# numz/ComfyUI-SeedVR2_VideoUpscaler

Hardware: AMD Instinct MI355X
Metric: upscaled frames/sec (720p->4K, SeedVR2-3B) (higher is better)
Workload: dtype bf16; 1 GPU; cfg3: SeedVR2-3B 32-frame 720p->4K clip (padded to 33 = 4n+1 for encode + DiT, 32 decoded), VAE tiled 1024/128; vae_tiled=True, parallelism=dp1, weights=random-init SeedVR2-3B + video_vae_v3 architecture (seeded)

## Files before the change

### comfyui-seedvr2_videoupscaler_amd/csrc/svr_conv_sub.hip

```cpp
#include "svr_common.h"
#include "../../include/seedvr2_hip.h"
#include <type_traits>

namespace svr {

constexpr int CS_TY = 16, CS_TX = 32, CS_HX = CS_TX + 1, CS_HY = CS_TY + 1;
constexpr int CS_NT = 256;
constexpr int CS_ROWS = CS_HX * CS_HY;
constexpr int CS_PIECES = (CS_ROWS * 4 + CS_NT - 1) / CS_NT;
constexpr int CS_ABUF = CS_PIECES * CS_NT * 16;
constexpr int CS_NBUF = 4;
constexpr int CS_EP_PITCH = 528;
constexpr int CS_EP_BYTES = 4 * 32 * CS_EP_PITCH;
constexpr int CS_LDS = CS_NBUF * CS_ABUF;
static_assert(CS_PIECES == 9 && CS_EP_BYTES <= CS_LDS, "piece schedule / epilogue parking");

template <int OFF> SVR_DEVICE void cs_rd2(bf16x8 (&r)[2], unsigned a0) {
    const unsigned a1 = a0 ^ 32u;
    asm volatile("ds_read_b128 %0, %2 offset:%4\n\tds_read_b128 %1, %3 offset:%4"
                 : "=&v"(r[0]), "=&v"(r[1]) : "v"(a0), "v"(a1), "n"(OFF) : "memory");
}
template <int N> SVR_DEVICE void cs_wait_rows(bf16x8 (&a)[2]) {
    asm volatile("s_waitcnt lgkmcnt(%2)" : "+v"(a[0]), "+v"(a[1]) : "n"(N));
    __builtin_amdgcn_sched_barrier(0);
}
template <int N> SVR_DEVICE void cs_wait_rows(bf16x8 (&a)[2], bf16x8 (&b)[2]) {
    asm volatile("s_waitcnt lgkmcnt(%4)" : "+v"(a[0]), "+v"(a[1]), "+v"(b[0]), "+v"(b[1]) : "n"(N));
    __builtin_amdgcn_sched_barrier(0);
}
template <int N> SVR_DEVICE void cs_wait_rows(bf16x8 (&a)[2], bf16x8 (&b)[2], bf16x8 (&c)[2], bf16x8 (&d)[2], bf16x8 (&e)[2]) {
    asm volatile("s_waitcnt lgkmcnt(%10)"
                 : "+v"(a[0]), "+v"(a[1]), "+v"(b[0]), "+v"(b[1]), "+v"(c[0]), "+v"(c[1]), "+v"(d[0]), "+v"(d[1]), "+v"(e[0]), "+v"(e[1])
                 : "n"(N));
    __builtin_amdgcn_sched_barrier(0);
}
template <int N> SVR_DEVICE void cs_wait_w(bf16x8 (&w)[2][2]) {
    asm volatile("s_waitcnt vmcnt(%4)" : "+v"(w[0][0]), "+v"(w[0][1]), "+v"(w[1][0]), "+v"(w[1][1]) : "n"(N));
    __builtin_amdgcn_sched_barrier(0);
}

__global__ __launch_bounds__(CS_NT, 1) void conv_sub_kernel(const svr_gemm_args a, const int band_rows) {
    constexpr int MTW = 8, NTW = 2, NT = CS_NT;
    extern __shared__ __attribute__((aligned(16))) char smem[];
    typedef __attribute__((ext_vector_type(16))) float f32x16_t;
    const svr_conv_geom& g = a.conv;
    const int tid = threadIdx.x;
    const int lane = tid & 63;
    const int wave = __builtin_amdgcn_readfirstlane(tid >> 6);
    const int wm = wave >> 1, wn = wave & 1;

    const int tiles_x = (g.W + CS_TX - 1) / CS_TX;
    const int tiles_y = (g.H + CS_TY - 1) / CS_TY;
    const int tiles_n = a.N / 128;
    int tl;
    {
        const int nwg = gridDim.x, bid = blockIdx.x;
        const int xcd = bid & 7, j = bid >> 3, q = nwg >> 3, r = nwg & 7;
        tl = (xcd < r ? xcd * (q + 1) : r * (q + 1) + (xcd - r) * q) + j;
    }
    const bool quad = a.phase.enabled && a.phase.quad != 0;
    int qp = 0;
    if (quad) { qp = tl & 3; tl >>= 2; }
    const int ph_py = quad ? (qp >> 1) : a.phase.py, ph_px = quad ? (qp & 1) : a.phase.px;
    const int pad_h = quad ? 1 - ph_py : g.ph, pad_w = quad ? 1 - ph_px : g.pw;
    const void* const w_frag = quad ? a.phase.W_frag4[qp] : a.W_frag;
    const float* const bias_p = quad ? a.phase.bias4[qp] : a.bias;
    const float* const bias_border_p = quad ? a.phase.bias_border4[qp] : a.phase.bias_border;
    const int tn = tl % tiles_n;
    int rr = tl / tiles_n;
    const int tx = rr % tiles_x; rr /= tiles_x;
    int ty, to;
    if (band_rows > 0 && band_rows < tiles_y) {
        const int per_band = band_rows * g.To;
        const int b = rr / per_band;
        const int rows_b = min(band_rows, tiles_y - b * band_rows);
        const int r2 = rr - b * per_band;
        to = r2 / rows_b;
        ty = b * band_rows + (r2 - to * rows_b);
    } else {
        ty = rr % tiles_y;
        to = rr / tiles_y;
    }
    const int y0 = ty * CS_TY, x0 = tx * CS_TX, n0 = tn * 128;

    const int cpk = g.Cin / 32;
    const int nA = g.kt * cpk;
    const int P = nA * 4;
    const int64_t frame_bytes = (int64_t)g.H * g.W * g.Cin * 2;
    const int srow = tid >> 2, spos = tid & 3;
    uint32_t poff[CS_PIECES];
    uint32_t akeys = 0;
#pragma unroll
    for (int q = 0; q < CS_PIECES; ++q) {
        const int row = q * (NT / 4) + srow;
        const int hy = row / CS_HX, hx = row - hy * CS_HX;
        const int y = y0 - pad_h + hy, x = x0 - pad_w + hx;
        const bool ok = (row < CS_ROWS) & ((unsigned)y < (unsigned)g.H) & ((unsigned)x < (unsigned)g.W);
        poff[q] = ok ? (uint32_t)(y * g.W + x) : 0xffffffffu;
        akeys |= (uint32_t)(spos ^ ((hx >> 2) & 3)) << (2 * q);
    }
    char* const wave_dst = smem + wave * 1024;
    auto frame_ptr = [&](int s) -> const char* {
        if (s >= nA) return nullptr;
        const int dt = s / cpk;
        const int c0 = (s - dt * cpk) * 32;
        int f = to + dt - g.pt;
        const char* basep = (const char*)a.A;
        if (f < 0) {
            if (g.halo != nullptr) { basep = (const char*)g.halo; f += g.halo_frames; }
            else f = 0;
        }
        return basep + (int64_t)f * frame_bytes + c0 * 2;
    };
    auto stage = [&](auto qc, const char* fptr, int buf) {
        constexpr int Q = decltype(qc)::value;
        const int ck = (akeys >> (2 * Q)) & 3;
        const char* src = (poff[Q] == 0xffffffffu || fptr == nullptr) ? (const char*)g.zeros
                                                                      : fptr + ((int64_t)poff[Q] * g.Cin + ck * 8) * 2;
        glds16(src, wave_dst + buf * CS_ABUF + Q * (NT * 16));
    };
    auto stage_all = [&](const char* fptr, int buf) {
        stage(std::integral_constant<int, 0>{}, fptr, buf); stage(std::integral_constant<int, 1>{}, fptr, buf);
        stage(std::integral_constant<int, 2>{}, fptr, buf); stage(std::integral_constant<int, 3>{}, fptr, buf);
        stage(std::integral_constant<int, 4>{}, fptr, buf); stage(std::integral_constant<int, 5>{}, fptr, buf);
        stage(std::integral_constant<int, 6>{}, fptr, buf); stage(std::integral_constant<int, 7>{}, fptr, buf);
        stage(std::integral_constant<int, 8>{}, fptr, buf);
    };

    const int l31 = lane & 31, hi = lane >> 5;
    const unsigned lds0 = (unsigned)(uintptr_t)(__attribute__((address_space(3))) char*)smem;
    unsigned fa[2];
#pragma unroll
    for (int dx = 0; dx < 2; ++dx)
        fa[dx] = lds0 + (unsigned)((wm * MTW * CS_HX + l31) * 64 + ((hi ^ (((dx + l31) >> 2) & 3)) << 4));

    f32x16_t acc[MTW][NTW];
#pragma unroll
    for (int y = 0; y < MTW; ++y)
#pragma unroll
        for (int z = 0; z < NTW; ++z)
#pragma unroll
            for (int e = 0; e < 16; ++e) acc[y][z][e] = 0.f;
    bf16x8 a0[2], a1[2], a2[2], a3[2], a4[2], a5[2], a6[2], a7[2], a8[2];
    bf16x8 w0[NTW][2], w1[NTW][2], w2[NTW][2], w3[NTW][2];

    const int64_t nstride = (int64_t)P * 2048;
    const char* wp0 = (const char*)w_frag + (int64_t)(n0 / 32 + wn * 2) * nstride;
    const char* wp1 = wp0 + nstride;
    const int voff = lane * 16;
    auto wload = [&](bf16x8 (&w)[NTW][2], int k) {
        auto uniform_ptr = [](const char* p) {
            const uint64_t u = (uint64_t)p;
            const uint32_t lo = __builtin_amdgcn_readfirstlane((uint32_t)u), hi_ = __builtin_amdgcn_readfirstlane((uint32_t)(u >> 32));
            return (const char*)(((uint64_t)hi_ << 32) | lo);
        };
        const char* p0 = uniform_ptr(wp0 + (int64_t)min(k, P - 1) * 2048);
        const char* p1 = uniform_ptr(wp1 + (int64_t)min(k, P - 1) * 2048);
        asm volatile("global_load_dwordx4 %0, %1, %2" : "=v"(w[0][0]) : "v"(voff), "s"(p0) : "memory");
        asm volatile("global_load_dwordx4 %0, %1, %2 offset:1024" : "=v"(w[0][1]) : "v"(voff), "s"(p0) : "memory");
        asm volatile("global_load_dwordx4 %0, %1, %2" : "=v"(w[1][0]) : "v"(voff), "s"(p1) : "memory");
        asm volatile("global_load_dwordx4 %0, %1, %2 offset:1024" : "=v"(w[1][1]) : "v"(voff), "s"(p1) : "memory");
    };

#define CS_RD(ROW, R, DXV, BUFOFF) cs_rd2<((R) * CS_HX + (DXV)) * 64>(ROW, fa[DXV] + (BUFOFF))
#define CS_MM(W, KS, ROW, MT, NTI) \
    acc[MT][NTI] = __builtin_amdgcn_mfma_f32_32x32x16_bf16(W[NTI][KS], ROW[KS], acc[MT][NTI], 0, 0, 0)
#define CS_MM8(W, RA, MA, RB, MB) \
    CS_MM(W, 0, RA, MA, 0); CS_MM(W, 0, RA, MA, 1); CS_MM(W, 0, RB, MB, 0); CS_MM(W, 0, RB, MB, 1); \
    CS_MM(W, 1, RA, MA, 0); CS_MM(W, 1, RA, MA, 1); CS_MM(W, 1, RB, MB, 0); CS_MM(W, 1, RB, MB, 1)

    auto interval = [&](auto jc, int s, const char* fstage, bf16x8 (&wc)[NTW][2], bf16x8 (&wn_)[NTW][2]) {
        constexpr int J = decltype(jc)::value;
        constexpr int DX = J >> 1, DY = J & 1;
        constexpr int NPC[4] = {0, 0, 5, 4};
        constexpr int NV = 4 + NPC[(J + 3) & 3] + NPC[(J + 2) & 3];
        const int k = s * 4 + J;
        const unsigned cur = (unsigned)((s & 3) * CS_ABUF), nxt = (unsigned)(((s + 1) & 3) * CS_ABUF);
        const int sbuf = (s + 3) & 3;
        constexpr int NDX = DX ^ 1;
        const unsigned nb = DX == 0 ? cur : nxt;
        if constexpr (DY == 0) {
            CS_RD(a8, 8, DX, cur);
            cs_wait_rows<8>(a0, a1, a2, a3, a4);
            cs_wait_w<NV>(wc);
            CS_MM8(wc, a0, 0, a1, 1);
            __builtin_amdgcn_sched_barrier(0);
            CS_RD(a0, 0, NDX, nb);
            wload(wn_, k + 2);
            __builtin_amdgcn_sched_barrier(0);
            CS_MM8(wc, a2, 2, a3, 3);
            __builtin_amdgcn_sched_barrier(0);
            if constexpr (J == 2) {
                stage(std::integral_constant<int, 0>{}, fstage, sbuf); stage(std::integral_constant<int, 1>{}, fstage, sbuf);
                stage(std::integral_constant<int, 2>{}, fstage, sbuf);
            }
            cs_wait_rows<8>(a4, a5);
            CS_MM8(wc, a4, 4, a5, 5);
            __builtin_amdgcn_sched_barrier(0);
            if constexpr (J == 2) { stage(std::integral_constant<int, 3>{}, fstage, sbuf); stage(std::integral_constant<int, 4>{}, fstage, sbuf); }
            cs_wait_rows<4>(a6, a7);
            CS_MM8(wc, a6, 6, a7, 7);
            __builtin_amdgcn_sched_barrier(0);
        } else {
            cs_wait_w<NV>(wc);
            CS_MM8(wc, a1, 0, a2, 1);
            __builtin_amdgcn_sched_barrier(0);
            CS_RD(a1, 1, NDX, nb); CS_RD(a2, 2, NDX, nb);
            wload(wn_, k + 2);
            __builtin_amdgcn_sched_barrier(0);
            CS_MM8(wc, a3, 2, a4, 3);
            __builtin_amdgcn_sched_barrier(0);
            CS_RD(a3, 3, NDX, nb); CS_RD(a4, 4, NDX, nb);
            if constexpr (J == 3) { stage(std::integral_constant<int, 5>{}, fstage, sbuf); stage(std::integral_constant<int, 6>{}, fstage, sbuf); }
            __builtin_amdgcn_sched_barrier(0);
            CS_MM8(wc, a5, 4, a6, 5);
            __builtin_amdgcn_sched_barrier(0);
            CS_RD(a5, 5, NDX, nb); CS_RD(a6, 6, NDX, nb);
            if constexpr (J == 3) { stage(std::integral_constant<int, 7>{}, fstage, sbuf); stage(std::integral_constant<int, 8>{}, fstage, sbuf); }
            cs_wait_rows<14>(a8);
            CS_MM8(wc, a7, 6, a8, 7);
            __builtin_amdgcn_sched_barrier(0);
            CS_RD(a7, 7, NDX, nb);
            if constexpr (J == 1) {
                __builtin_amdgcn_s_barrier();
                __builtin_amdgcn_sched_barrier(0);
            }
        }
    };

    stage_all(frame_ptr(0), 0);
    stage_all(frame_ptr(1), 1);
    stage_all(frame_ptr(2), 2);
    wload(w0, 0);
    wload(w1, 1);
    __builtin_amdgcn_sched_barrier(0);
#pragma unroll
    for (int y = 0; y < MTW; ++y)
#pragma unroll
        for (int z = 0; z < NTW; ++z) asm volatile("" : "+a"(acc[y][z]));
    asm volatile("s_waitcnt vmcnt(0)" ::: "memory");
    __builtin_amdgcn_s_barrier();
    __builtin_amdgcn_sched_barrier(0);
    CS_RD(a0, 0, 0, 0u); CS_RD(a1, 1, 0, 0u); CS_RD(a2, 2, 0, 0u); CS_RD(a3, 3, 0, 0u);
    CS_RD(a4, 4, 0, 0u); CS_RD(a5, 5, 0, 0u); CS_RD(a6, 6, 0, 0u); CS_RD(a7, 7, 0, 0u);

    for (int s = 0; s < nA; ++s) {
        const char* fs = frame_ptr(s + 3);
        interval(std::integral_constant<int, 0>{}, s, fs, w0, w2);
        interval(std::integral_constant<int, 1>{}, s, fs, w1, w3);
        interval(std::integral_constant<int, 2>{}, s, fs, w2, w0);
        interval(std::integral_constant<int, 3>{}, s, fs, w3, w1);
    }
    asm volatile("s_waitcnt vmcnt(0) lgkmcnt(0)" ::: "memory");
    __builtin_amdgcn_sched_barrier(0);
    __syncthreads();
#undef CS_RD
#undef CS_MM
#undef CS_MM8

    const int hi4 = hi * 4;
    const int n = n0 + (tid & 15) * 8;
    f32x4 bias_lo = {0.f, 0.f, 0.f, 0.f}, bias_hi = {0.f, 0.f, 0.f, 0.f};
    if (bias_p) {
        bias_lo = *(const f32x4*)(bias_p + n);
        bias_hi = *(const f32x4*)(bias_p + n + 4);
    }
    const int py = a.phase.enabled ? ph_py : 0, px = a.phase.enabled ? ph_px : 0;
    const int up = a.phase.enabled ? 2 : 1, ts = a.phase.enabled ? a.phase.t_stride : 1;
    const int yb = py ? g.H - 1 : 0, xb = px ? g.W - 1 : 0;
    const float* btab = a.phase.enabled ? bias_border_p : nullptr;
    double gs0 = 0.0, gq0 = 0.0, gs1 = 0.0, gq1 = 0.0;
    auto ep_body = [&](auto o32c) {
    constexpr int OKIND = decltype(o32c)::value;
    constexpr bool O32 = OKIND == SVR_STORE_FP32;
#pragma unroll
    for (int pass = 0; pass < MTW / 2; ++pass) {
        __builtin_amdgcn_sched_barrier(0);
#pragma unroll
        for (int j = 0; j < 2; ++j) {
            char* row = smem + ((wm * 2 + j) * 32 + l31) * CS_EP_PITCH;
#pragma unroll
            for (int nt = 0; nt < NTW; ++nt) {
                const f32x16_t v = acc[2 * pass + j][nt];
#pragma unroll
                for (int gq = 0; gq < 4; ++gq) {
                    const f32x4 o = {v[4 * gq], v[4 * gq + 1], v[4 * gq + 2], v[4 * gq + 3]};
                    *(f32x4*)(row + (wn * 64 + nt * 32 + 8 * gq + hi4) * 4) = o;
                }
            }
        }
        lds_barrier();
#pragma unroll
        for (int half = 0; half < 2; ++half) {
            f32x4 lo[4], hi_[4];
            int64_t off[4];
            bool ok[4];
            int border[4];
#pragma unroll
            for (int it = 0; it < 4; ++it) {
                const int vox = ((half * 4 + it) * NT + tid) >> 4;
                const int r = vox >> 5;
                const int y = y0 + (r >> 1) * MTW + 2 * pass + (r & 1), x = x0 + (vox & 31);
                ok[it] = y < g.H && x < g.W;
                const int yc = min(y, g.H - 1), xc = min(x, g.W - 1);
                border[it] = (yc == yb ? 1 : 0) | (xc == xb ? 2 : 0);
                off[it] = (((int64_t)to * ts * (up * g.H) + up * yc + py) * (up * g.W) + up * xc + px) * a.N + n;
                lo[it] = *(const f32x4*)(smem + vox * CS_EP_PITCH + (tid & 15) * 32);
                hi_[it] = *(const f32x4*)(smem + vox * CS_EP_PITCH + (tid & 15) * 32 + 16);
            }
#pragma unroll
            for (int it = 0; it < 4; ++it) {
                f32x4 bl = bias_lo, bh = bias_hi;
                if (btab != nullptr && border[it] != 0) {
                    const float* bb = btab + (int64_t)(border[it] - 1) * a.N + n;
                    bl = *(const f32x4*)bb;
                    bh = *(const f32x4*)(bb + 4);
                }
                const float f[8] = {lo[it][0] + bl[0], lo[it][1] + bl[1], lo[it][2] + bl[2], lo[it][3] + bl[3],
                                    hi_[it][0] + bh[0], hi_[it][1] + bh[1], hi_[it][2] + bh[2], hi_[it][3] + bh[3]};
                float r[8];
                if constexpr (O32) {
                    if (ok[it]) {
                        float* cp = (float*)a.C + off[it];
                        *(float4*)cp = make_float4(f[0], f[1], f[2], f[3]);
                        *(float4*)(cp + 4) = make_float4(f[4], f[5], f[6], f[7]);
                    }
#pragma unroll
                    for (int e = 0; e < 8; ++e) r[e] = f[e];
                } else {
                    const uint4 pk = OKIND == SVR_STORE_H16 ? pack8h(f) : pack8(f);
                    if (ok[it]) *(uint4*)((bf16_t*)a.C + off[it]) = pk;
                    if constexpr (OKIND == SVR_STORE_H16) unpack8h(pk, r); else unpack8(pk, r);
                }
                if (a.gn_partial != nullptr && ok[it]) {
                    gn_accumulate4(gs0, gq0, r[0], r[1], r[2], r[3]);
                    gn_accumulate4(gs1, gq1, r[4], r[5], r[6], r[7]);
                }
            }
        }
        if (pass + 1 < MTW / 2) lds_barrier();
    }
    };
    if (a.out_f32 == SVR_STORE_FP32) ep_body(std::integral_constant<int, SVR_STORE_FP32>{});
    else if (a.out_f32 == SVR_STORE_H16) ep_body(std::integral_constant<int, SVR_STORE_H16>{});
    else ep_body(std::integral_constant<int, SVR_STORE_BF16>{});
    if (a.gn_partial) {
        __syncthreads();
        double4* red = (double4*)smem;
        double2* qsum = (double2*)(smem + NT * 32);
        red[tid] = make_double4(gs0, gq0, gs1, gq1);
        __syncthreads();
        if (tid < 32) {
            const int c = tid >> 1, h = tid & 1;
            double s_ = 0.0, q_ = 0.0;
            for (int j = 0; j < NT / 16; ++j) {
                const double4 v = red[(j << 4) | c];
                s_ += h ? v.z : v.x;
                q_ += h ? v.w : v.y;
            }
            qsum[tid] = make_double2(s_, q_);
        }
        __syncthreads();
        const int qpg = (a.N / a.gn_groups) >> 2;
        if (tid < 32 / qpg) {
            double s_ = 0.0, q_ = 0.0;
            for (int i = 0; i < qpg; ++i) { s_ += qsum[tid * qpg + i].x; q_ += qsum[tid * qpg + i].y; }
            const int nblk = tiles_y * tiles_x;
            const int per_frame = a.phase.enabled ? 4 * nblk : nblk;
            const int slot = (a.phase.enabled ? (py * 2 + px) * nblk : 0) + ty * tiles_x + tx;
            ((double2*)a.gn_partial)[((int64_t)to * ts * per_frame + slot) * a.gn_groups + (n0 >> 2) / qpg + tid] = make_double2(s_, q_);
        }
    }
}

int g_conv_sub = 1;

static bool conv_sub_gn_ok(const svr_gemm_args& a) {
    const int cpg = a.gn_groups > 0 ? a.N / a.gn_groups : 0;
    return cpg >= 4 && !(cpg & 3) && a.N % a.gn_groups == 0 && 128 % cpg == 0;
}

static bool conv_sub_eligible(const svr_gemm_args& a) {
    const svr_conv_geom& g = a.conv;
    const bool quad = a.phase.enabled && a.phase.quad != 0;
    bool ptrs = true;
    if (quad) {
        for (int p = 0; p < 4; ++p)
            ptrs = ptrs && a.phase.W_frag4[p] != nullptr && (!a.phase.bias4[p] || ((uintptr_t)a.phase.bias4[p] % 16) == 0) &&
                   (!a.phase.bias_border4[p] || ((uintptr_t)a.phase.bias_border4[p] % 16) == 0);
    } else {
        ptrs = a.W_frag != nullptr && (unsigned)g.ph <= 1u && (unsigned)g.pw <= 1u && (!a.bias || ((uintptr_t)a.bias % 16) == 0) &&
               (!a.phase.bias_border || ((uintptr_t)a.phase.bias_border % 16) == 0);
    }
    return g_conv_sub && g.enabled && ptrs && g.kh == 2 && g.kw == 2 && g.sh == 1 && g.sw == 1 && g.st == 1 &&
           g.Ho == g.H && g.Wo == g.W && g.Cin % 32 == 0 && g.kt >= 1 && g.kt <= 3 &&
           g.To == g.T + g.pt - g.kt + 1 && !a.ps.enabled && a.epilogue == SVR_EPI_BIAS && !a.resid && !a.gate &&
           (!a.gn_partial || conv_sub_gn_ok(a)) && (a.N % 128) == 0 && (a.phase.enabled || (a.ldc == a.N)) &&
           (int64_t)g.H * g.W * g.Cin * 2 < (int64_t)1 << 32 && ((uintptr_t)a.C % 16) == 0;
}

static int conv_sub_gn_blocks(const svr_gemm_args& a) {
    if (!conv_sub_eligible(a) || !conv_sub_gn_ok(a)) return 0;
    const int nblk = ((a.conv.H + CS_TY - 1) / CS_TY) * ((a.conv.W + CS_TX - 1) / CS_TX);
    return a.phase.enabled ? 4 * nblk : nblk;
}

static int launch_conv_sub(const svr_gemm_args& a, hipStream_t s) {
    const svr_conv_geom& g = a.conv;
    const int tiles = g.To * ((g.H + CS_TY - 1) / CS_TY) * ((g.W + CS_TX - 1) / CS_TX) * (a.N / 128) *
                      (a.phase.enabled && a.phase.quad ? 4 : 1);
    static uint64_t lds_attr_done = 0;
    {
        const int e = set_max_dynamic_lds((const void*)conv_sub_kernel, 160 * 1024, lds_attr_done);
        if (e != 0) return e;
    }
    hipLaunchKernelGGL(conv_sub_kernel, dim3(tiles), dim3(CS_NT), CS_LDS, s, a, g_conv_band);
    return (int)hipGetLastError();
}

__global__ __launch_bounds__(256) void conv_pack_frag_taps_kernel(const bf16_t* __restrict__ W, uint4* __restrict__ out, int N, int K,
                                                                  int kt, int kh, int kw, int Cin) {
    const int cpk = Cin / 32, taps = kh * kw, P = kt * cpk * taps;
    const int64_t idx = (int64_t)blockIdx.x * 256 + threadIdx.x;
    if (idx >= (int64_t)(N / 32) * P * 128) return;
    const int lane = (int)(idx & 63), ks = (int)((idx >> 6) & 1);
    const int kk = (int)((idx >> 7) % P), n32 = (int)((idx >> 7) / P);
    const int s = kk / taps, J = kk - s * taps;
    const int dt = s / cpk, cs = s - dt * cpk, dy = J % kh, dx = J / kh;
    const int nn = n32 * 32 + (lane & 31), c = cs * 32 + ks * 16 + (lane >> 5) * 8;
    out[idx] = *(const uint4*)(W + (int64_t)nn * K + ((dt * kh + dy) * kw + dx) * Cin + c);
}

}
```

Before: 3.827 frames/s.

## Switch conv_sub inner product from 32x32x16 to 16x16x32 MFMA tiles

```diff
diff --git a/comfyui-seedvr2_videoupscaler_amd/csrc/svr_conv_sub.hip b/comfyui-seedvr2_videoupscaler_amd/csrc/svr_conv_sub.hip
--- a/comfyui-seedvr2_videoupscaler_amd/csrc/svr_conv_sub.hip
+++ b/comfyui-seedvr2_videoupscaler_amd/csrc/svr_conv_sub.hip
@@ -16,9 +16,15 @@
 static_assert(CS_PIECES == 9 && CS_EP_BYTES <= CS_LDS, "piece schedule / epilogue parking");
 
 template <int OFF> SVR_DEVICE void cs_rd2(bf16x8 (&r)[2], unsigned a0) {
-    const unsigned a1 = a0 ^ 32u;
-    asm volatile("ds_read_b128 %0, %2 offset:%4\n\tds_read_b128 %1, %3 offset:%4"
-                 : "=&v"(r[0]), "=&v"(r[1]) : "v"(a0), "v"(a1), "n"(OFF) : "memory");
+    static_assert(OFF >= 0 && OFF + 1024 + 16 <= 65536, "ds_read offset field");
+    asm volatile("ds_read_b128 %0, %2 offset:%3\n\tds_read_b128 %1, %2 offset:%4"
+                 : "=&v"(r[0]), "=&v"(r[1]) : "v"(a0), "n"(OFF), "n"(OFF + 1024) : "memory");
+}
+SVR_DEVICE void cs_mm4(f32x4 (&c)[2][2], const bf16x8 (&w)[2], const bf16x8 (&r)[2]) {
+    c[0][0] = __builtin_amdgcn_mfma_f32_16x16x32_bf16(w[0], r[0], c[0][0], 0, 0, 0);
+    c[0][1] = __builtin_amdgcn_mfma_f32_16x16x32_bf16(w[1], r[0], c[0][1], 0, 0, 0);
+    c[1][0] = __builtin_amdgcn_mfma_f32_16x16x32_bf16(w[0], r[1], c[1][0], 0, 0, 0);
+    c[1][1] = __builtin_amdgcn_mfma_f32_16x16x32_bf16(w[1], r[1], c[1][1], 0, 0, 0);
 }
 template <int N> SVR_DEVICE void cs_wait_rows(bf16x8 (&a)[2]) {
     asm volatile("s_waitcnt lgkmcnt(%2)" : "+v"(a[0]), "+v"(a[1]) : "n"(N));
@@ -42,7 +48,6 @@
 __global__ __launch_bounds__(CS_NT, 1) void conv_sub_kernel(const svr_gemm_args a, const int band_rows) {
     constexpr int MTW = 8, NTW = 2, NT = CS_NT;
     extern __shared__ __attribute__((aligned(16))) char smem[];
-    typedef __attribute__((ext_vector_type(16))) float f32x16_t;
     const svr_conv_geom& g = a.conv;
     const int tid = threadIdx.x;
     const int lane = tid & 63;
@@ -127,27 +132,27 @@
         stage(std::integral_constant<int, 8>{}, fptr, buf);
     };
 
-    const int l31 = lane & 31, hi = lane >> 5;
+    const int l15 = lane & 15, c4 = lane >> 4;
     const unsigned lds0 = (unsigned)(uintptr_t)(__attribute__((address_space(3))) char*)smem;
     unsigned fa[2];
 #pragma unroll
     for (int dx = 0; dx < 2; ++dx)
-        fa[dx] = lds0 + (unsigned)((wm * MTW * CS_HX + l31) * 64 + ((hi ^ (((dx + l31) >> 2) & 3)) << 4));
-
-    f32x16_t acc[MTW][NTW];
+        fa[dx] = lds0 + (unsigned)((wm * MTW * CS_HX + l15) * 64 + ((c4 ^ (((dx + l15) >> 2) & 3)) << 4));
+
+    f32x4 acc[MTW][NTW][2][2];
 #pragma unroll
     for (int y = 0; y < MTW; ++y)
 #pragma unroll
         for (int z = 0; z < NTW; ++z)
 #pragma unroll
-            for (int e = 0; e < 16; ++e) acc[y][z][e] = 0.f;
+            for (int e = 0; e < 4; ++e) acc[y][z][e >> 1][e & 1] = f32x4{0.f, 0.f, 0.f, 0.f};
     bf16x8 a0[2], a1[2], a2[2], a3[2], a4[2], a5[2], a6[2], a7[2], a8[2];
     bf16x8 w0[NTW][2], w1[NTW][2], w2[NTW][2], w3[NTW][2];
 
     const int64_t nstride = (int64_t)P * 2048;
     const char* wp0 = (const char*)w_frag + (int64_t)(n0 / 32 + wn * 2) * nstride;
     const char* wp1 = wp0 + nstride;
-    const int voff = lane * 16;
+    const int voff = c4 * 512 + l15 * 16;
     auto wload = [&](bf16x8 (&w)[NTW][2], int k) {
         auto uniform_ptr = [](const char* p) {
             const uint64_t u = (uint64_t)p;
@@ -157,17 +162,14 @@
         const char* p0 = uniform_ptr(wp0 + (int64_t)min(k, P - 1) * 2048);
         const char* p1 = uniform_ptr(wp1 + (int64_t)min(k, P - 1) * 2048);
         asm volatile("global_load_dwordx4 %0, %1, %2" : "=v"(w[0][0]) : "v"(voff), "s"(p0) : "memory");
-        asm volatile("global_load_dwordx4 %0, %1, %2 offset:1024" : "=v"(w[0][1]) : "v"(voff), "s"(p0) : "memory");
+        asm volatile("global_load_dwordx4 %0, %1, %2 offset:256" : "=v"(w[0][1]) : "v"(voff), "s"(p0) : "memory");
         asm volatile("global_load_dwordx4 %0, %1, %2" : "=v"(w[1][0]) : "v"(voff), "s"(p1) : "memory");
-        asm volatile("global_load_dwordx4 %0, %1, %2 offset:1024" : "=v"(w[1][1]) : "v"(voff), "s"(p1) : "memory");
+        asm volatile("global_load_dwordx4 %0, %1, %2 offset:256" : "=v"(w[1][1]) : "v"(voff), "s"(p1) : "memory");
     };
 
 #define CS_RD(ROW, R, DXV, BUFOFF) cs_rd2<((R) * CS_HX + (DXV)) * 64>(ROW, fa[DXV] + (BUFOFF))
-#define CS_MM(W, KS, ROW, MT, NTI) \
-    acc[MT][NTI] = __builtin_amdgcn_mfma_f32_32x32x16_bf16(W[NTI][KS], ROW[KS], acc[MT][NTI], 0, 0, 0)
 #define CS_MM8(W, RA, MA, RB, MB) \
-    CS_MM(W, 0, RA, MA, 0); CS_MM(W, 0, RA, MA, 1); CS_MM(W, 0, RB, MB, 0); CS_MM(W, 0, RB, MB, 1); \
-    CS_MM(W, 1, RA, MA, 0); CS_MM(W, 1, RA, MA, 1); CS_MM(W, 1, RB, MB, 0); CS_MM(W, 1, RB, MB, 1)
+    cs_mm4(acc[MA][0], W[0], RA); cs_mm4(acc[MA][1], W[1], RA); cs_mm4(acc[MB][0], W[0], RB); cs_mm4(acc[MB][1], W[1], RB)
 
     auto interval = [&](auto jc, int s, const char* fstage, bf16x8 (&wc)[NTW][2], bf16x8 (&wn_)[NTW][2]) {
         constexpr int J = decltype(jc)::value;
@@ -237,7 +239,8 @@
 #pragma unroll
     for (int y = 0; y < MTW; ++y)
 #pragma unroll
-        for (int z = 0; z < NTW; ++z) asm volatile("" : "+a"(acc[y][z]));
+        for (int z = 0; z < NTW; ++z)
+            asm volatile("" : "+a"(acc[y][z][0][0]), "+a"(acc[y][z][0][1]), "+a"(acc[y][z][1][0]), "+a"(acc[y][z][1][1]));
     asm volatile("s_waitcnt vmcnt(0)" ::: "memory");
     __builtin_amdgcn_s_barrier();
     __builtin_amdgcn_sched_barrier(0);
@@ -255,10 +258,8 @@
     __builtin_amdgcn_sched_barrier(0);
     __syncthreads();
 #undef CS_RD
-#undef CS_MM
 #undef CS_MM8
 
-    const int hi4 = hi * 4;
     const int n = n0 + (tid & 15) * 8;
     f32x4 bias_lo = {0.f, 0.f, 0.f, 0.f}, bias_hi = {0.f, 0.f, 0.f, 0.f};
     if (bias_p) {
@@ -278,15 +279,14 @@
         __builtin_amdgcn_sched_barrier(0);
 #pragma unroll
         for (int j = 0; j < 2; ++j) {
-            char* row = smem + ((wm * 2 + j) * 32 + l31) * CS_EP_PITCH;
-#pragma unroll
-            for (int nt = 0; nt < NTW; ++nt) {
-                const f32x16_t v = acc[2 * pass + j][nt];
-#pragma unroll
-                for (int gq = 0; gq < 4; ++gq) {
-                    const f32x4 o = {v[4 * gq], v[4 * gq + 1], v[4 * gq + 2], v[4 * gq + 3]};
-                    *(f32x4*)(row + (wn * 64 + nt * 32 + 8 * gq + hi4) * 4) = o;
-                }
+#pragma unroll
+            for (int vh = 0; vh < 2; ++vh) {
+                char* row = smem + ((wm * 2 + j) * 32 + vh * 16 + l15) * CS_EP_PITCH;
+#pragma unroll
+                for (int nt = 0; nt < NTW; ++nt)
+#pragma unroll
+                    for (int ch = 0; ch < 2; ++ch)
+                        *(f32x4*)(row + (wn * 64 + nt * 32 + ch * 16 + c4 * 4) * 4) = acc[2 * pass + j][nt][vh][ch];
             }
         }
         lds_barrier();
```

Result: no change. 3.852 frames/s, median of 6 (+0.7%).
